# rokulkarni15/distributed-llm-training-inference

Hardware: AMD Instinct MI355X
Metric: train tok/s Llama-2-7B ZeRO-3+LoRA at 1/2/4/8 GPUs; serve tok/s + p50 TTFT (higher is better)
Workload: dtype bf16

## Files before the change

lumen/csrc/kernels/flash_attn.hip:

```cpp
#include "api.h"
#include "common.h"
#include <cstdlib>

namespace lumen {
namespace fa {

typedef __bf16 bf16x8 __attribute__((ext_vector_type(8)));
typedef _Float16 f16x8 __attribute__((ext_vector_type(8)));
typedef float f32x4 __attribute__((ext_vector_type(4)));
typedef short s16x4 __attribute__((ext_vector_type(4)));
typedef __attribute__((address_space(3))) s16x4 lds_s16x4;

constexpr int D = 128;
constexpr int BN = 64;
constexpr int IMG = BN * D * 2;

template <typename T> struct Mfma;
template <> struct Mfma<bf16> {
  static __device__ __forceinline__ f32x4 run(uint4 a, uint4 b, f32x4 c) {
    return __builtin_amdgcn_mfma_f32_16x16x32_bf16(__builtin_bit_cast(bf16x8, a),
                                                   __builtin_bit_cast(bf16x8, b), c, 0, 0, 0);
  }
};
template <> struct Mfma<fp16> {
  static __device__ __forceinline__ f32x4 run(uint4 a, uint4 b, f32x4 c) {
    return __builtin_amdgcn_mfma_f32_16x16x32_f16(__builtin_bit_cast(f16x8, a),
                                                  __builtin_bit_cast(f16x8, b), c, 0, 0, 0);
  }
};

__device__ __forceinline__ int swz(int row) { return ((row & 3) << 2) | ((row >> 2) & 3); }
__device__ __forceinline__ int img_off(int row, int chunk) {
  return row * 256 + ((chunk ^ swz(row)) << 4);
}
template <int SW>
__device__ __forceinline__ int swz_t(int row) {
  if constexpr (SW == 0) return swz(row);
  else return ((row & 1) << 3) | ((row & 2) << 1) | ((row & 4) >> 1);
}
__device__ __forceinline__ unsigned lds_off_g(const char* p) {
  return static_cast<unsigned>(
      reinterpret_cast<uintptr_t>((__attribute__((address_space(3))) const char*)(p)));
}
template <int SW>
__device__ __forceinline__ int img_off_t(int row, int chunk) {
  return row * 256 + ((chunk ^ swz_t<SW>(row)) << 4);
}

template <typename T>
__device__ __forceinline__ void stage64(char* img, const T* base, long long ld, int r0, int rmax) {
#pragma unroll
  for (int i = 0; i < 4; ++i) {
    const int idx = threadIdx.x + i * 256;
    const int row = idx >> 4, ch = idx & 15;
    uint4 v = make_uint4(0, 0, 0, 0);
    if (r0 + row < rmax) v = *reinterpret_cast<const uint4*>(base + (long long)(r0 + row) * ld + ch * 8);
    *reinterpret_cast<uint4*>(img + img_off(row, ch)) = v;
  }
}

template <typename T, int SW = 0>
__device__ __forceinline__ void stage64_async(char* img, const T* base, long long ld, int r0,
                                              int rmax) {
  const int lane = threadIdx.x & 63, wid = threadIdx.x >> 6;
#pragma unroll
  for (int i = 0; i < 4; ++i) {
    const int row = (wid * 4 + i) * 4 + (lane >> 4);
    const int ch = (lane & 15) ^ swz_t<SW>(row);
    int gr = r0 + row;
    gr = gr < rmax ? gr : rmax - 1;
    __builtin_amdgcn_global_load_lds(
        (const void*)(base + (long long)gr * ld + ch * 8),
        (__attribute__((address_space(3))) void*)(img + (wid * 4 + i) * 1024), 16, 0, 0);
  }
}

template <typename T>
__device__ __forceinline__ void stage64_async_s(char* img, const T* base, long long ld, int r0,
                                                int rmax) {
  const int lane = threadIdx.x & 63, wid = __builtin_amdgcn_readfirstlane(threadIdx.x >> 6);
  const char* tile = reinterpret_cast<const char*>(base + (long long)r0 * ld);
  const int last = rmax - 1 - r0;
#pragma unroll
  for (int i = 0; i < 4; ++i) {
    const int row = (wid * 4 + i) * 4 + (lane >> 4);
    const int ch = (lane & 15) ^ swz(row);
    const unsigned off = (unsigned)((row < last ? row : last) * (int)ld + ch * 8) * sizeof(T);
    __builtin_amdgcn_global_load_lds(
        (const void*)(tile + off),
        (__attribute__((address_space(3))) void*)(img + (wid * 4 + i) * 1024), 16, 0, 0);
  }
}

__device__ __forceinline__ void dma16_o(const void* g, const char* lds_wave_base) {
  const unsigned m0 = __builtin_amdgcn_readfirstlane(lds_off_g(lds_wave_base));
  asm volatile("s_mov_b32 m0, %1\n\ts_nop 0\n\tglobal_load_lds_dwordx4 %0, off"
               :: "v"(g), "s"(m0) : "memory", "m0");
}
__device__ __forceinline__ void dma4_o(const void* g, const char* lds_wave_base) {
  const unsigned m0 = __builtin_amdgcn_readfirstlane(lds_off_g(lds_wave_base));
  asm volatile("s_mov_b32 m0, %1\n\ts_nop 0\n\tglobal_load_lds_dword %0, off"
               :: "v"(g), "s"(m0) : "memory", "m0");
}
template <typename T, int SW>
__device__ __forceinline__ void stage64_async_o(char* img, const T* base, long long ld, int r0,
                                                int rmax) {
  const int lane = threadIdx.x & 63, wid = __builtin_amdgcn_readfirstlane(threadIdx.x >> 6);
#pragma unroll
  for (int i = 0; i < 4; ++i) {
    const int row = (wid * 4 + i) * 4 + (lane >> 4);
    const int ch = (lane & 15) ^ swz_t<SW>(row);
    int gr = r0 + row;
    gr = gr < rmax ? gr : rmax - 1;
    dma16_o(base + (long long)gr * ld + ch * 8, img + (wid * 4 + i) * 1024);
  }
}

template <typename T, int SW>
__device__ __forceinline__ void stage64_async8_o(char* img, const T* base, long long ld, int r0,
                                                 int rmax) {
  const int lane = threadIdx.x & 63, wid = threadIdx.x >> 6;
#pragma unroll
  for (int i = 0; i < 2; ++i) {
    const int row = (wid * 2 + i) * 4 + (lane >> 4);
    const int ch = (lane & 15) ^ swz_t<SW>(row);
    int gr = r0 + row;
    gr = gr < rmax ? gr : rmax - 1;
    dma16_o(base + (long long)gr * ld + ch * 8, img + (wid * 2 + i) * 1024);
  }
}

template <typename T>
__device__ __forceinline__ void stage64_paged(char* img, const T* cache, int kvh, int nkv,
                                              const int* bt, int bs, int r0, int rmax) {
  const int lane = threadIdx.x & 63, wid = threadIdx.x >> 6;
#pragma unroll
  for (int i = 0; i < 4; ++i) {
    const int row = (wid * 4 + i) * 4 + (lane >> 4);
    const int ch = (lane & 15) ^ swz(row);
    int gr = r0 + row;
    gr = gr < rmax ? gr : rmax - 1;
    const long long blk = bt[gr / bs];
    const T* src = cache + ((blk * nkv + kvh) * bs + gr % bs) * D + ch * 8;
    __builtin_amdgcn_global_load_lds(
        (const void*)src, (__attribute__((address_space(3))) void*)(img + (wid * 4 + i) * 1024),
        16, 0, 0);
  }
}

__device__ __forceinline__ void wait_vm_all() { __builtin_amdgcn_s_waitcnt(0xF70); }
__device__ __forceinline__ void wait_vm_8() { __builtin_amdgcn_s_waitcnt(0xF78); }
__device__ __forceinline__ void lds_fence_barrier() {
  asm volatile("s_waitcnt lgkmcnt(0)" ::: "memory");
  __builtin_amdgcn_s_barrier();
  asm volatile("" ::: "memory");
}

template <int SW = 0>
__device__ __forceinline__ uint4 row_read(const char* img, int row, int chunk) {
  return *reinterpret_cast<const uint4*>(img + img_off_t<SW>(row, chunk));
}

__device__ __forceinline__ uint2 tr_read_raw(const char* p) {
  s16x4 r = __builtin_amdgcn_ds_read_tr16_b64_v4i16((lds_s16x4*)(p));
  return __builtin_bit_cast(uint2, r);
}

__device__ __forceinline__ uint4 tr_read_img(const char* img, int k0, int n0, int lane) {
  const int L = lane & 15, g = lane >> 4;
  const int col = n0 + 4 * (L & 3);
  const int ch = col >> 3, half = (col >> 2) & 1;
  const int r = k0 + 8 * g + (L >> 2);
  const uint2 lo = tr_read_raw(img + img_off(r, ch) + 8 * half);
  const uint2 hi = tr_read_raw(img + img_off(r + 4, ch) + 8 * half);
  return make_uint4(lo.x, lo.y, hi.x, hi.y);
}

__device__ __forceinline__ uint4 tr_read_y(const char* y, int cols, int k0, int m0, int lane) {
  const int L = lane & 15, g = lane >> 4;
  const int r = k0 + 8 * g + (L >> 2);
  const int c = m0 + 4 * (L & 3);
  const int ld = cols + 4;
  const uint2 lo = tr_read_raw(y + (r * ld + c) * 2);
  const uint2 hi = tr_read_raw(y + ((r + 4) * ld + c) * 2);
  return make_uint4(lo.x, lo.y, hi.x, hi.y);
}

template <typename T>
__device__ __forceinline__ void y_store(char* y, int cols, int k0, int m0, int lane, float v0,
                                        float v1, float v2, float v3) {
  T t[4] = {from_f32<T>(v0), from_f32<T>(v1), from_f32<T>(v2), from_f32<T>(v3)};
  *reinterpret_cast<uint2*>(y + ((k0 + (lane & 15)) * (cols + 4) + m0 + 4 * (lane >> 4)) * 2) =
      *reinterpret_cast<uint2*>(t);
}

template <typename T>
__device__ __forceinline__ uint4 gload16(const T* p, bool ok) {
  return ok ? *reinterpret_cast<const uint4*>(p) : make_uint4(0, 0, 0, 0);
}

template <int CTRL>
__device__ __forceinline__ float dpp(float v) {
  return __builtin_bit_cast(float, __builtin_amdgcn_update_dpp(0, __builtin_bit_cast(int, v), CTRL,
                                                               0xF, 0xF, false));
}
__device__ __forceinline__ float red16_max(float v) {
  v = fmaxf(v, dpp<0xB1>(v));
  v = fmaxf(v, dpp<0x4E>(v));
  v = fmaxf(v, dpp<0x141>(v));
  v = fmaxf(v, dpp<0x140>(v));
  return v;
}
__device__ __forceinline__ float red16_sum(float v) {
  v += dpp<0xB1>(v);
  v += dpp<0x4E>(v);
  v += dpp<0x141>(v);
  v += dpp<0x140>(v);
  return v;
}

__device__ __forceinline__ float fexp2(float x) { return __builtin_amdgcn_exp2f(x); }

struct Args {
  const void* q; const void* k; const void* v;
  long long ldq, ldk, ldv;
  void* o; long long ldo;
  float* lse;
  const int* cu;
  const int* tiles;
  int nh, nkv, T;
  float scale, scale_log2;
  const void* dout; long long lddo;
  void* dq; void* dk; void* dv; long long lddq, lddk, lddv;
  const float* delta;
  const int* rope_pos;
  const float* rope_cos;
  const float* rope_sin;
  const int* kv_lens;
  const int* block_tables;
  int bt_stride;
  int block_size;
  void* ds;
  const int* ds_off;
  int ds_total;
  int tiles3;
  int nitems;
  int snake;
};

struct Work { int seq, r0, head; };
__device__ __forceinline__ Work work_item(const Args& a) {
  if (a.tiles3) {
    const int* t = a.tiles + 3 * blockIdx.x;
    return Work{t[0], t[1], t[2]};
  }
  return Work{a.tiles[2 * blockIdx.x], a.tiles[2 * blockIdx.x + 1], (int)blockIdx.y};
}

__device__ __forceinline__ void rope_inv_pair(float& lo, float& hi, float c, float s) {
  const float l = lo, h = hi;
  lo = l * c + h * s;
  hi = h * c - l * s;
}

template <int SW = 0>
__device__ __forceinline__ uint4 tr_read_img2(const char* img, int rlo, int rhi, int n0, int lane) {
  const int L = lane & 15;
  const int col = n0 + 4 * (L & 3);
  const int ch = col >> 3, half = (col >> 2) & 1;
  const uint2 lo = tr_read_raw(img + img_off_t<SW>(rlo + (L >> 2), ch) + 8 * half);
  const uint2 hi = tr_read_raw(img + img_off_t<SW>(rhi + (L >> 2), ch) + 8 * half);
  return make_uint4(lo.x, lo.y, hi.x, hi.y);
}

template <typename T>
__device__ __forceinline__ uint4 pack_p(const f32x4& a, const f32x4& b) {
  return make_uint4(pk2<T>(a[0], a[1]), pk2<T>(a[2], a[3]), pk2<T>(b[0], b[1]), pk2<T>(b[2], b[3]));
}

template <typename T>
__global__ void __launch_bounds__(256) delta_kernel(Args a) {
  const int lane = threadIdx.x & 63;
  const int t = blockIdx.x * 4 + (threadIdx.x >> 6);
  if (t >= a.T) return;
  const int H = a.nh * D;
  const T* dO = reinterpret_cast<const T*>(a.dout) + (long long)t * a.lddo;
  const T* O = reinterpret_cast<const T*>(a.o) + (long long)t * a.ldo;
  for (int base = 0; base < H; base += 512) {
    const int e = base + lane * 8;
    float s = 0.f;
    if (e < H) {
      float x[8], y[8];
      load8(dO + e, x);
      load8(O + e, y);
#pragma unroll
      for (int j = 0; j < 8; ++j) s += x[j] * y[j];
    }
#pragma unroll
    for (int o = 1; o < 16; o <<= 1) s += __shfl_xor(s, o, 16);
    if ((lane & 15) == 0 && e < H) const_cast<float*>(a.delta)[(long long)(e / D) * a.T + t] = s;
  }
}

__device__ __forceinline__ int ds_slot(int m, int lr) { return (m * 16 + (lr ^ ((m & 1) << 3))) * 16; }
__device__ __forceinline__ long long ds_tile(const Args& a, int head, int seq_base, int qt, int kt,
// ... 305 lines not shown
    vr[1][n] = tr32a<1>(vb, off, n);
    vr[2][n] = tr32a<2>(vb, off, n);
    vr[3][n] = tr32a<3>(vb, off, n);
  }
  float mx = -INFINITY;
#pragma unroll
  for (int kb = 0; kb < 2; ++kb)
#pragma unroll
    for (int r = 0; r < 16; ++r) {
      if (MASK) {
        const int kpos = kv0 + kb * 32 + 8 * (r >> 2) + 4 * hi + (r & 3);
        const bool out = (kpos >= L) | (CAUSAL & (kpos > qrow));
        st[kb][r] = out ? -INFINITY : st[kb][r];
      }
      mx = fmaxf(mx, st[kb][r]);
    }
  mx = xor32_max(mx) * scale_log2;
  constexpr float RESCALE = 8.f;
  const bool bump = mx > m_i + RESCALE;
  if (__any(bump)) {
    const float alpha = bump ? fexp2(m_i - mx) : 1.f;
    const float m_new = bump ? mx : m_i;
    l_i *= alpha;
#pragma unroll
    for (int n = 0; n < 4; ++n) acc[n] *= alpha;
    m_i = m_new;
  }
  const float mref = m_i == -INFINITY ? 0.f : m_i;
  float rs = 0.f;
#pragma unroll
  for (int kb = 0; kb < 2; ++kb)
#pragma unroll
    for (int r = 0; r < 16; ++r) {
      const float p = fexp2(fmaf(st[kb][r], scale_log2, -mref));
      st[kb][r] = p;
      rs += p;
    }
  l_i += xor32_sum(rs);
  const uint4 pb[4] = {pack8<T>(st[0], 0), pack8<T>(st[0], 1), pack8<T>(st[1], 0),
                       pack8<T>(st[1], 1)};
#pragma unroll
  for (int sl = 0; sl < 4; ++sl) {
    lgkm_wait(vr[sl][0], vr[sl][1], vr[sl][2], vr[sl][3]);
#pragma unroll
    for (int n = 0; n < 4; ++n) acc[n] = Mfma32<T>::run(as_u4(vr[sl][n]), pb[sl], acc[n]);
  }
}

template <typename T, bool CAUSAL, bool PAGED = false>
__global__ void __launch_bounds__(256, CAUSAL ? 2 : 1) fwd32_kernel(Args a) {
  constexpr int BM = 128;
  __shared__ __attribute__((aligned(16))) char bufA[2 * IMG];
  __shared__ __attribute__((aligned(16))) char bufB[2 * IMG];
  const int lane = threadIdx.x & 63, wid = threadIdx.x >> 6;
  const int lq = lane & 31, hi = lane >> 5;
  auto run = [&](const int seq, const int q0, const int head) {
  const int kvh = head / (a.nh / a.nkv);
  const int s0 = a.cu[seq], L = a.cu[seq + 1] - s0;
  const int Lk = PAGED ? a.kv_lens[seq] : L;
  const int qoff = Lk - L;
  const T* Q = reinterpret_cast<const T*>(a.q) + (long long)s0 * a.ldq + head * D;
  const T* K = reinterpret_cast<const T*>(a.k) + (PAGED ? 0 : (long long)s0 * a.ldk + kvh * D);
  const T* V = reinterpret_cast<const T*>(a.v) + (PAGED ? 0 : (long long)s0 * a.ldv + kvh * D);
  const int* bt = PAGED ? a.block_tables + (long long)seq * a.bt_stride : nullptr;
  const int wq0 = q0 + wid * 32;
  const int qrow = wq0 + lq;
  const int qpos = qrow + qoff;
  Off32 off;
  make_off32(off, lane);
  f32x16 acc[4];
#pragma unroll
  for (int n = 0; n < 4; ++n) acc[n] = zero16();
  float m_i = -INFINITY, l_i = 0.f;
  const int kv_end = CAUSAL ? min(Lk, q0 + qoff + BM) : Lk;
  const int w_end = CAUSAL ? min(kv_end, wq0 + qoff + 32) : kv_end;
  auto stage = [&](char* img, int r0) {
    if constexpr (PAGED) {
      stage64_paged(img, K, kvh, a.nkv, bt, a.block_size, r0, Lk);
      stage64_paged(img + IMG, V, kvh, a.nkv, bt, a.block_size, r0, Lk);
    } else {
      stage64_async_s(img, K, a.ldk, r0, L);
      stage64_async_s(img + IMG, V, a.ldv, r0, L);
    }
  };
  uint4 qf[8];
  {
    const bool two = q0 + 64 < L;
    stage64_async_s(bufB, Q, a.ldq, q0, L);
    if (two) stage64_async_s(bufB + IMG, Q, a.ldq, q0 + 64, L);
    if (kv_end > 0) {
      stage(bufA, 0);
      wait_vm_8();
    } else {
      wait_vm_all();
    }
    __builtin_amdgcn_s_barrier();
    asm volatile("" ::: "memory");
    const int r = 32 * wid + lq;
    const char* qi = bufB + (r >> 6) * IMG;
#pragma unroll
    for (int ks = 0; ks < 8; ++ks) qf[ks] = row_read(qi, r & 63, 2 * ks + hi);
    lds_fence_barrier();
  }
  auto tile = [&](char* cur, char* nxt, int kv0) {
    if (kv0 + BN < kv_end) {
      stage(nxt, kv0 + BN);
      wait_vm_8();
    } else {
      wait_vm_all();
    }
    lds_fence_barrier();
    if (kv0 < w_end) {
      const bool need_mask = (kv0 + BN > Lk) || (CAUSAL && kv0 + BN - 1 > wq0 + qoff);
      if (need_mask)
        fwd32_tile<T, CAUSAL, true>(cur, cur + IMG, off, qf, acc, m_i, l_i, kv0, Lk, qpos,
                                           hi, a.scale_log2);
      else
        fwd32_tile<T, CAUSAL, false>(cur, cur + IMG, off, qf, acc, m_i, l_i, kv0, Lk, qpos,
                                            hi, a.scale_log2);
    }
    lds_fence_barrier();
  };
  for (int kv0 = 0; kv0 < kv_end; kv0 += 2 * BN) {
    tile(bufA, bufB, kv0);
    if (kv0 + BN < kv_end) tile(bufB, bufA, kv0 + BN);
  }
  {
    int ln = threadIdx.x;
    asm volatile("" : "+v"(ln));
    const int lq2 = ln & 31, hi2 = (ln >> 5) & 1;
    const float inv = l_i > 0.f ? 1.f / l_i : 0.f;
    char* ot = bufA + wid * 8192;
#pragma unroll
    for (int n = 0; n < 4; ++n)
#pragma unroll
      for (int j = 0; j < 4; ++j) {
        struct alignas(8) O4 { T v[4]; } o4;
#pragma unroll
        for (int i = 0; i < 4; ++i) o4.v[i] = from_f32<T>(acc[n][4 * j + i] * inv);
        *reinterpret_cast<O4*>(ot + img_off(lq2, 4 * n + j) + 8 * hi2) = o4;
      }
    if (hi == 0 && a.lse && qrow < L)
      a.lse[(long long)head * a.T + s0 + qrow] = l_i > 0.f ? m_i + __log2f(l_i) : INFINITY;
    asm volatile("s_waitcnt lgkmcnt(0)" ::: "memory");
    T* O = reinterpret_cast<T*>(a.o) + (long long)s0 * a.ldo + head * D;
    const int ch = ln & 15;
#pragma unroll
    for (int it = 0; it < 8; ++it) {
      const int r = 4 * it + ((ln >> 4) & 3);
      const uint4 v = *reinterpret_cast<const uint4*>(ot + img_off(r, ch));
      if (wq0 + r < L) *reinterpret_cast<uint4*>(O + (long long)(wq0 + r) * a.ldo + ch * 8) = v;
    }
  }
  if (a.nitems > 0) lds_fence_barrier();
  };
  if (a.nitems > 0) {
    const int G = gridDim.x, w = blockIdx.x;
    for (int base = 0; base < a.nitems; base += G) {
      const int it = (a.snake && ((base / G) & 1)) ? base + G - 1 - w : base + w;
      if (it >= a.nitems) continue;
      const int ti = it / a.nh;
      run(a.tiles[2 * ti], a.tiles[2 * ti + 1], it - ti * a.nh);
    }
  } else {
    const Work wk = work_item(a);
    if (wk.seq < 0) return;
    run(wk.seq, wk.r0, wk.head);
  }
}


template <typename T, bool CAUSAL, bool MASK>
__device__ __forceinline__ void dq32_tile(const char* kimg, const char* vimg, const Off32& off,
                                          const uint4 (&qf)[8], const uint4 (&of)[8],
                                          f32x16 (&dq)[4], int kv0, int L, int qrow, int hi,
                                          float lse_q, float del_q, float scale_log2) {
#pragma unroll
  for (int kb = 0; kb < 2; ++kb) {
    f32x16 st = zero16(), dpt = zero16();
#pragma unroll
    for (int ks = 0; ks < 8; ++ks) {
      st = Mfma32<T>::run(lds16(kimg + kb * 8192 + off.row[ks]), qf[ks], st);
      dpt = Mfma32<T>::run(lds16(vimg + kb * 8192 + off.row[ks]), of[ks], dpt);
    }
#pragma unroll
    for (int r = 0; r < 16; ++r) {
      float pv = fexp2(fmaf(st[r], scale_log2, -lse_q));
      if (MASK) {
        const int kpos = kv0 + kb * 32 + 8 * (r >> 2) + 4 * hi + (r & 3);
        const bool out = (kpos >= L) | (qrow >= L) | (CAUSAL & (kpos > qrow));
        pv = out ? 0.f : pv;
      }
      dpt[r] = pv * (dpt[r] - del_q);
    }
#pragma unroll
    for (int s = 0; s < 2; ++s) {
      const uint4 db = pack8<T>(dpt, s);
#pragma unroll
      for (int n = 0; n < 4; ++n)
        dq[n] = Mfma32<T>::run(tr32(kimg, off, kb * 32 + 16 * s, n), db, dq[n]);
    }
  }
}

template <typename T, bool CAUSAL>
__global__ void __launch_bounds__(256, 2) bwd_dq32_kernel(Args a) {
  constexpr int BM = 128;
  __shared__ __attribute__((aligned(16))) char smem[4 * IMG];
  const int lane = threadIdx.x & 63, wid = threadIdx.x >> 6;
  const int lq = lane & 31, hi = lane >> 5;
  const Work wk = work_item(a);
  if (wk.seq < 0) return;
  const int seq = wk.seq, q0 = wk.r0;
  const int head = wk.head, kvh = head / (a.nh / a.nkv);
  const int s0 = a.cu[seq], L = a.cu[seq + 1] - s0;
  const T* Q = reinterpret_cast<const T*>(a.q) + (long long)s0 * a.ldq + head * D;
  const T* dO = reinterpret_cast<const T*>(a.dout) + (long long)s0 * a.lddo + head * D;
  const T* K = reinterpret_cast<const T*>(a.k) + (long long)s0 * a.ldk + kvh * D;
  const T* V = reinterpret_cast<const T*>(a.v) + (long long)s0 * a.ldv + kvh * D;
  const int wq0 = q0 + wid * 32;
  const int qrow = wq0 + lq;
  uint4 qf[8], of[8];
#pragma unroll
  for (int ks = 0; ks < 8; ++ks) {
    qf[ks] = gload16(Q + (long long)qrow * a.ldq + 16 * ks + 8 * hi, qrow < L);
    of[ks] = gload16(dO + (long long)qrow * a.lddo + 16 * ks + 8 * hi, qrow < L);
  }
  const float lse_q = qrow < L ? a.lse[(long long)head * a.T + s0 + qrow] : INFINITY;
  const float del_q = qrow < L ? a.delta[(long long)head * a.T + s0 + qrow] : 0.f;
  f32x16 dq[4];
#pragma unroll
  for (int n = 0; n < 4; ++n) dq[n] = zero16();
  const int kv_end = CAUSAL ? min(L, q0 + BM) : L;
  const int w_end = CAUSAL ? min(kv_end, wq0 + 32) : kv_end;
  wait_vm_all();
  if (kv_end > 0) {
    stage64_async(smem, K, a.ldk, 0, L);
    stage64_async(smem + IMG, V, a.ldv, 0, L);
  }
  Off32 off;
  make_off32(off, lane);
  int it = 0;
  for (int kv0 = 0; kv0 < kv_end; kv0 += BN, ++it) {
    char* kimg = smem + (it & 1) * 2 * IMG;
    char* vimg = kimg + IMG;
    if (kv0 + BN < kv_end) {
      char* nk = smem + ((it + 1) & 1) * 2 * IMG;
      stage64_async(nk, K, a.ldk, kv0 + BN, L);
      stage64_async(nk + IMG, V, a.ldv, kv0 + BN, L);
      wait_vm_8();
    } else {
      wait_vm_all();
    }
    lds_fence_barrier();
    if (kv0 < w_end) {
      const bool need_mask = (kv0 + BN > L) || (wq0 + 32 > L) || (CAUSAL && kv0 + BN - 1 > wq0);
      if (need_mask)
        dq32_tile<T, CAUSAL, true>(kimg, vimg, off, qf, of, dq, kv0, L, qrow, hi, lse_q, del_q,
                                   a.scale_log2);
      else
        dq32_tile<T, CAUSAL, false>(kimg, vimg, off, qf, of, dq, kv0, L, qrow, hi, lse_q, del_q,
                                    a.scale_log2);
    }
    lds_fence_barrier();
  }
  if (qrow < L) {
    T* dQ = reinterpret_cast<T*>(a.dq) + (long long)s0 * a.lddq + head * D + (long long)qrow * a.lddq;
#pragma unroll
    for (int n = 0; n < 4; ++n)
#pragma unroll
      for (int r = 0; r < 16; ++r) dq[n][r] *= a.scale;
    if (a.rope_pos != nullptr) {
      const float* cb = a.rope_cos + (long long)a.rope_pos[s0 + qrow] * 64 + 4 * hi;
      const float* sb = a.rope_sin + (long long)a.rope_pos[s0 + qrow] * 64 + 4 * hi;
#pragma unroll
      for (int n = 0; n < 2; ++n)
#pragma unroll
        for (int jj = 0; jj < 4; ++jj) {
          const float4 c4 = *reinterpret_cast<const float4*>(cb + 32 * n + 8 * jj);
          const float4 s4 = *reinterpret_cast<const float4*>(sb + 32 * n + 8 * jj);
          const float cs[4] = {c4.x, c4.y, c4.z, c4.w}, sn[4] = {s4.x, s4.y, s4.z, s4.w};
#pragma unroll
          for (int i = 0; i < 4; ++i) {
            float lo = dq[n][4 * jj + i], hi2 = dq[n + 2][4 * jj + i];
            rope_inv_pair(lo, hi2, cs[i], sn[i]);
            dq[n][4 * jj + i] = lo;
            dq[n + 2][4 * jj + i] = hi2;
          }
        }
    }
#pragma unroll
    for (int n = 0; n < 4; ++n)
#pragma unroll
      for (int jj = 0; jj < 4; ++jj) {
        struct alignas(8) O4 { T v[4]; } q4;
#pragma unroll
        for (int i = 0; i < 4; ++i) q4.v[i] = from_f32<T>(dq[n][4 * jj + i]);
        *reinterpret_cast<O4*>(dQ + 32 * n + 8 * jj + 4 * hi) = q4;
      }
  }
}

template <typename T, bool CAUSAL>
__global__ void __launch_bounds__(256) bwd_dq_ds_kernel(Args a) {
  constexpr int TILE = IMG + 8192;
  __shared__ __attribute__((aligned(16))) char bufA[TILE];
  __shared__ __attribute__((aligned(16))) char bufB[TILE];
  const int lane = threadIdx.x & 63, wid = __builtin_amdgcn_readfirstlane(threadIdx.x >> 6);
  const int lr = lane & 15, lg = lane >> 4;
  auto run = [&](const int seq, const int q0, const int head) {
  const int kvh = head / (a.nh / a.nkv);
  const int s0 = a.cu[seq], L = a.cu[seq + 1] - s0;
  const int ns = (L + 63) / 64, qt = q0 / 64;
  const T* K = reinterpret_cast<const T*>(a.k) + (long long)s0 * a.ldk + kvh * D;
  const char* dsq = reinterpret_cast<const char*>(a.ds) + ds_tile(a, head, a.ds_off[seq], qt, 0, ns, CAUSAL);
  const int nkt = CAUSAL ? qt + 1 : ns;
  const int si = lr >> 2, sm = lr & 3;
  const int dso = ((wid >> 1) * 1024) + (wid & 1) * 8 + ds_slot(sm, 4 * lg + si);
  auto stage = [&](char* buf, int kt) {
    stage64_async_o<T, 1>(buf, K, a.ldk, kt * 64, L);
    const char* src = dsq + (long long)kt * 8192;
#pragma unroll
    for (int i = 0; i < 2; ++i) {
      const int off = (wid * 2 + i) * 1024;
      dma16_o(src + off + lane * 16, buf + IMG + off);
    }
  };
  f32x4 dq[8];
#pragma unroll
  for (int n = 0; n < 8; ++n) dq[n] = f32x4{0.f, 0.f, 0.f, 0.f};
  if (nkt > 0) stage(bufA, 0);
  auto step = [&](int kt, char* buf, char* nx) {
    if (kt + 1 < nkt) {
      stage(nx, kt + 1);
      asm volatile("s_waitcnt vmcnt(6)" ::: "memory");
    } else {
      wait_vm_all();
    }
    lds_fence_barrier();
    const char* kimg = buf;
    const char* dsi = buf + IMG;
#pragma unroll
    for (int ks = 0; ks < 2; ++ks) {
      const uint2 lo = tr_read_raw(dsi + (2 * ks) * 2048 + dso);
      const uint2 hi = tr_read_raw(dsi + (2 * ks + 1) * 2048 + dso);
      const uint4 af = make_uint4(lo.x, lo.y, hi.x, hi.y);
#pragma unroll
      for (int n = 0; n < 8; ++n)
        dq[n] = Mfma<T>::run(af, tr_read_img2<1>(kimg, 32 * ks + 4 * lg, 32 * ks + 16 + 4 * lg, n * 16, lane), dq[n]);
    }
    lds_fence_barrier();
  };
  for (int kt = 0; kt < nkt; kt += 2) {
    step(kt, bufA, bufB);
    if (kt + 1 < nkt) step(kt + 1, bufB, bufA);
  }
  T* dQ = reinterpret_cast<T*>(a.dq) + (long long)s0 * a.lddq + head * D;
#pragma unroll
  for (int r = 0; r < 4; ++r) {
    const int qr = q0 + wid * 16 + 4 * lg + r;
    if (qr >= L) continue;
    float qv[8];
#pragma unroll
    for (int n = 0; n < 8; ++n) qv[n] = dq[n][r] * a.scale;
    if (a.rope_pos != nullptr) {
      const long long pb = (long long)a.rope_pos[s0 + qr] * 64 + lr;
#pragma unroll
      for (int n = 0; n < 4; ++n)
        rope_inv_pair(qv[n], qv[n + 4], a.rope_cos[pb + 16 * n], a.rope_sin[pb + 16 * n]);
    }
#pragma unroll
    for (int n = 0; n < 8; ++n) dQ[(long long)qr * a.lddq + n * 16 + lr] = from_f32<T>(qv[n]);
  }
  };
  if (a.nitems > 0) {
    const int G = gridDim.x, w = blockIdx.x;
    for (int base = 0; base < a.nitems; base += G) {
      const int it = (a.snake && ((base / G) & 1)) ? base + G - 1 - w : base + w;
      if (it >= a.nitems) continue;
      const int ti = it / a.nh;
      run(a.tiles[2 * ti], a.tiles[2 * ti + 1], it - ti * a.nh);
    }
  } else {
    const Work wk = work_item(a);
    if (wk.seq < 0) return;
    run(wk.seq, wk.r0, wk.head);
  }
}


static int cu_count() {
  static int n = [] {
    int dev = 0, v = 0;
    if (hipGetDevice(&dev) != hipSuccess ||
        hipDeviceGetAttribute(&v, hipDeviceAttributeMultiprocessorCount, dev) != hipSuccess || v <= 0)
      v = 256;
    return v;
  }();
  return n;
}

template <typename T>
static hipError_t launch(int which, int causal, int mt, int ntiles, const Args& a, hipStream_t st) {
  dim3 block(256);
  if (which == 0) {
    if (mt != 20) return hipErrorInvalidValue;
    dim3 grid(ntiles, a.tiles3 ? 1 : a.nh);
    if (a.nitems > 0) grid = dim3(std::min(a.nitems, (causal ? 2 : 1) * cu_count()), 1);
    if (causal) hipLaunchKernelGGL((fwd32_kernel<T, true>), grid, block, 0, st, a);
    else hipLaunchKernelGGL((fwd32_kernel<T, false>), grid, block, 0, st, a);
  } else if (which == 1) {
    dim3 grid((unsigned)((a.T + 3) / 4));
    hipLaunchKernelGGL(delta_kernel<T>, grid, block, 0, st, a);
  } else if (which == 2) {
    dim3 grid(ntiles, a.tiles3 ? 1 : a.nkv);
    if (causal) hipLaunchKernelGGL((bwd_dkdv_kernel<T, true>), grid, block, 0, st, a);
    else hipLaunchKernelGGL((bwd_dkdv_kernel<T, false>), grid, block, 0, st, a);
  } else if (which == 5) {
    dim3 grid(ntiles, a.tiles3 ? 1 : a.nh);
    if (causal) hipLaunchKernelGGL((bwd_dq32_kernel<T, true>), grid, block, 0, st, a);
    else hipLaunchKernelGGL((bwd_dq32_kernel<T, false>), grid, block, 0, st, a);
  } else if (which == 7) {
    dim3 grid(ntiles, a.tiles3 ? 1 : a.nkv);
    if (a.nitems > 0) grid = dim3(std::min(a.nitems, 2 * cu_count()), 1);
    if (causal) hipLaunchKernelGGL((bwd_dkdv_kernel<T, true, true>), grid, block, 0, st, a);
    else hipLaunchKernelGGL((bwd_dkdv_kernel<T, false, true>), grid, block, 0, st, a);
  } else if (which == 8) {
    dim3 grid(ntiles, a.tiles3 ? 1 : a.nh);
    if (a.nitems > 0) grid = dim3(std::min(a.nitems, 3 * cu_count()), 1);
    if (causal) hipLaunchKernelGGL((bwd_dq_ds_kernel<T, true>), grid, block, 0, st, a);
    else hipLaunchKernelGGL((bwd_dq_ds_kernel<T, false>), grid, block, 0, st, a);
  } else if (which == 6) {
    dim3 grid(ntiles, a.nh);
    if (a.nitems > 0) grid = dim3(std::min(a.nitems, (causal ? 2 : 1) * cu_count()), 1);
    if (causal) hipLaunchKernelGGL((fwd32_kernel<T, true, true>), grid, block, 0, st, a);
    else hipLaunchKernelGGL((fwd32_kernel<T, false, true>), grid, block, 0, st, a);
  } else {
    return hipErrorInvalidValue;
  }
  return hipGetLastError();
}

}
}

#include <algorithm>
#include <cstdlib>
static int fa_persist() {
  static int v = [] { const char* e = std::getenv("LUMEN_FA_PERSIST"); return e ? std::atoi(e) : 15; }();
  return v;
}

extern "C" hipError_t lumen_flash_attn(int dtype, int which, int causal, int mt,
                                       const void* q, const void* k, const void* v,
                                       long long ldq, long long ldk, long long ldv, void* o,
                                       long long ldo, float* lse, const int* cu,
                                       const int* tiles, int ntiles, int nh, int nkv, int T,
                                       float scale, const void* dout, long long lddo, void* dq,
                                       void* dk, void* dv, long long lddq, long long lddk,
                                       long long lddv, const float* delta, const int* rope_pos,
                                       const float* rope_cos, const float* rope_sin,
                                       hipStream_t st) {
  if (nkv <= 0 || nh % nkv != 0) return hipErrorInvalidValue;
  const int tiles3 = (which >> 8) & 1;
  which &= 0xff;
  if (tiles3 && which != 0 && which != 2 && which != 5) return hipErrorInvalidValue;
  if (rope_pos != nullptr && which != 2 && which != 5) return hipErrorInvalidValue;
  if (which != 1 && ntiles == 0) return hipSuccess;
  lumen::fa::Args a;
  a.q = q; a.k = k; a.v = v; a.ldq = ldq; a.ldk = ldk; a.ldv = ldv; a.o = o; a.ldo = ldo;
  a.lse = lse; a.cu = cu; a.tiles = tiles; a.nh = nh; a.nkv = nkv; a.T = T;
  a.scale = scale; a.scale_log2 = scale * 1.4426950408889634f;
  a.dout = dout; a.lddo = lddo; a.dq = dq; a.dk = dk; a.dv = dv; a.lddq = lddq; a.lddk = lddk;
  a.lddv = lddv; a.delta = delta;
  a.rope_pos = rope_pos; a.rope_cos = rope_cos; a.rope_sin = rope_sin;
  a.kv_lens = nullptr; a.block_tables = nullptr; a.bt_stride = 0; a.block_size = 0;
  a.ds = nullptr; a.ds_off = nullptr; a.ds_total = 0; a.tiles3 = tiles3;
  a.nitems = (which == 0 && mt == 20 && !tiles3 && (fa_persist() & 2)) ? ntiles * nh : 0;
  a.snake = (fa_persist() >> 3) & 1;
  if (which == 6 || which == 7 || which == 8) return hipErrorInvalidValue;
  if (dtype == lumen::kBF16) return lumen::fa::launch<lumen::bf16>(which, causal, mt, ntiles, a, st);
  if (dtype == lumen::kF16) return lumen::fa::launch<lumen::fp16>(which, causal, mt, ntiles, a, st);
  return hipErrorInvalidValue;
}

extern "C" hipError_t lumen_flash_attn_paged(int dtype, int causal, const void* q, long long ldq,
                                             const void* k_cache, const void* v_cache, void* o,
                                             long long ldo, const int* cu_q, const int* kv_lens,
                                             const int* tiles, int ntiles,
                                             const int* block_tables, int bt_stride,
                                             int block_size, int nh, int nkv, int T, float scale,
                                             hipStream_t st) {
  if (nkv <= 0 || nh % nkv != 0 || block_size <= 0) return hipErrorInvalidValue;
  if (ntiles == 0) return hipSuccess;
  lumen::fa::Args a{};
  a.q = q; a.ldq = ldq; a.k = k_cache; a.v = v_cache; a.ldk = a.ldv = 0;
  a.o = o; a.ldo = ldo; a.lse = nullptr; a.cu = cu_q; a.tiles = tiles;
  a.nh = nh; a.nkv = nkv; a.T = T;
  a.scale = scale; a.scale_log2 = scale * 1.4426950408889634f;
  a.kv_lens = kv_lens; a.block_tables = block_tables; a.bt_stride = bt_stride;
  a.block_size = block_size;
  a.nitems = 0;
  if (dtype == lumen::kBF16) return lumen::fa::launch<lumen::bf16>(6, causal, 20, ntiles, a, st);
  if (dtype == lumen::kF16) return lumen::fa::launch<lumen::fp16>(6, causal, 20, ntiles, a, st);
  return hipErrorInvalidValue;
}

extern "C" hipError_t lumen_flash_attn_ds(int dtype, int which, int causal, const void* q,
                                          const void* k, const void* v, long long ldq,
                                          long long ldk, long long ldv, const float* lse,
                                          const int* cu, const int* tiles, int ntiles, int nh,
                                          int nkv, int T, float scale, const void* dout,
                                          long long lddo, void* dq, void* dk, void* dv,
                                          long long lddq, long long lddk, long long lddv,
                                          const float* delta, const int* rope_pos,
                                          const float* rope_cos, const float* rope_sin, void* ds,
                                          const int* ds_off, int ds_total, hipStream_t st) {
  const int tiles3 = (which >> 8) & 1;
  which &= 0xff;
  if (nkv <= 0 || nh % nkv != 0 || (which != 7 && which != 8) || ds == nullptr ||
      ds_off == nullptr)
    return hipErrorInvalidValue;
  if (ntiles == 0) return hipSuccess;
  lumen::fa::Args a{};
  a.q = q; a.k = k; a.v = v; a.ldq = ldq; a.ldk = ldk; a.ldv = ldv;
  a.lse = const_cast<float*>(lse); a.cu = cu; a.tiles = tiles; a.nh = nh; a.nkv = nkv; a.T = T;
  a.scale = scale; a.scale_log2 = scale * 1.4426950408889634f;
  a.dout = dout; a.lddo = lddo; a.dq = dq; a.dk = dk; a.dv = dv; a.lddq = lddq; a.lddk = lddk;
  a.lddv = lddv; a.delta = delta;
  a.rope_pos = rope_pos; a.rope_cos = rope_cos; a.rope_sin = rope_sin;
  a.ds = ds; a.ds_off = ds_off; a.ds_total = ds_total; a.tiles3 = tiles3;
  a.snake = (fa_persist() >> 3) & 1;
  a.nitems = tiles3 ? 0 : (which == 7 && (fa_persist() & 1)) ? ntiles * nkv
                        : (which == 8 && (fa_persist() & 4)) ? ntiles * nh : 0;
  if (dtype == lumen::kBF16) return lumen::fa::launch<lumen::bf16>(which, causal, 1, ntiles, a, st);
  if (dtype == lumen::kF16) return lumen::fa::launch<lumen::fp16>(which, causal, 1, ntiles, a, st);
  return hipErrorInvalidValue;
}
```

lumen/ops/attention.py:

```python
from __future__ import annotations

import math
import os
from typing import Optional

import torch
import torch.nn.functional as F

from ._native import native, use_native
from .quant import MX_BLOCK, Mxfp4Weight, quantize_mxfp4_rows


def causal_attention(q: torch.Tensor, k: torch.Tensor, v: torch.Tensor,
                     scale: Optional[float] = None) -> torch.Tensor:
    B, nh, S, D = q.shape
    nkv = k.shape[1]
    if nkv != nh:
        if q.is_cuda:
            o = F.scaled_dot_product_attention(q, k, v, is_causal=True, scale=scale,
                                               enable_gqa=True)
        else:
            rep = nh // nkv
            o = F.scaled_dot_product_attention(q, k.repeat_interleave(rep, 1),
                                               v.repeat_interleave(rep, 1), is_causal=True,
# ... 95 lines not shown
            to = torch.empty(num_seqs, nh, max_parts, D, device=q.device, dtype=torch.float32)
        else:
            tm = torch.empty(1, 1, 1, device=q.device, dtype=torch.float32)
            tl, to = tm, tm
        one = PA_ONE_PASS if one_pass is None else int(one_pass)
        fused = bool(fused_merge) and not one
        cnt = (_pa_counters(q.device, num_seqs * nkv) if fused and max_parts > 1
               else None)
        qk = q if (q.stride(2) == 1 and q.stride(1) == D and q.stride(0) % D == 0
                   and q.data_ptr() % 16 == 0) else q.contiguous()
        native().paged_attention_decode(out, qk, _kv_buf(k_cache), _kv_buf(v_cache), block_tables,
                                        context_lens, nkv, bs, block_tables.shape[1], scale, tm,
                                        tl, to, partition_size, cnt, one)
        return out
    return paged_decode_ref(q, k_cache, v_cache, block_tables, context_lens, scale)


def paged_decode_ref(q, k_cache, v_cache, block_tables, context_lens, scale):
    num_seqs, nh, D = q.shape
    nkv, bs = k_cache.shape[1], k_cache.shape[2]
    g = nh // nkv
    out = torch.empty_like(q)
    for i in range(num_seqs):
        L = int(context_lens[i])
        nblk = (L + bs - 1) // bs
        blks = block_tables[i, :nblk].long()
        kk = _kv_gather_f32(k_cache, blks).permute(1, 0, 2, 3).reshape(nkv, nblk * bs, D)[:, :L]
        vv = _kv_gather_f32(v_cache, blks).permute(1, 0, 2, 3).reshape(nkv, nblk * bs, D)[:, :L]
        qq = q[i].float().view(nkv, g, D)
        s = torch.einsum("hgd,hld->hgl", qq, kk) * scale
        p = torch.softmax(s, -1)
        out[i] = torch.einsum("hgl,hld->hgd", p, vv).reshape(nh, D).to(q.dtype)
    return out


def flash_attention_paged(q: torch.Tensor, k_cache: torch.Tensor, v_cache: torch.Tensor,
                          cu_q, kv_lens, block_tables: torch.Tensor, nh: int, nkv: int,
                          D: int, scale: Optional[float] = None,
                          out: Optional[torch.Tensor] = None) -> torch.Tensor:
    T = q.shape[0]
    scale = scale if scale is not None else 1.0 / math.sqrt(D)
    if out is None:
        out = torch.empty(T, nh * D, device=q.device, dtype=q.dtype)
    if use_native(q) and D == 128 and k_cache.shape[-1] == 128:
        cu = tuple(int(c) for c in cu_q)
        dev = q.device
        cut = _cu_tensor(cu, dev)
        kl = (kv_lens if isinstance(kv_lens, torch.Tensor)
              else torch.tensor(list(kv_lens), dtype=torch.int32, device=dev))
        kl = kl.to(torch.int32)
        bt = block_tables.to(torch.int32)
        if isinstance(k_cache, Mxfp4KV) or k_cache.dtype == FP8_KV:
            k_cache, v_cache, bt = _dequant_blocks(k_cache, v_cache, bt, kl, q.dtype)
        native().flash_attn_paged(True, q, k_cache, v_cache, out, cut, kl,
                                  _tiles(cu, 128, dev), bt, nh, nkv, scale)
        return out
    out.copy_(flash_attention_paged_ref(q, k_cache, v_cache, cu_q, kv_lens, block_tables, nh,
                                        nkv, D, scale))
    return out


FP8_KV = torch.float8_e4m3fn
_SCRATCH: dict = {}


def _dequant_blocks(k_cache, v_cache, bt, kv_lens, dtype):
    P, maxb = bt.shape
    nb, nkv, bs, D = k_cache.shape
    need = P * maxb
    key = (k_cache.device, dtype, nkv, bs, D)
    scr = _SCRATCH.get(key)
    if scr is None or scr[0].shape[0] < need:
        n = max(need, 256)
        scr = (torch.empty(n, nkv, bs, D, device=k_cache.device, dtype=dtype),
               torch.empty(n, nkv, bs, D, device=k_cache.device, dtype=dtype),
               torch.arange(n, device=k_cache.device, dtype=torch.int32))
        _SCRATCH[key] = scr
    ks, vs, ident = scr
    if isinstance(k_cache, Mxfp4KV):
        native().kv_dequant_mx(k_cache.buf, v_cache.buf, ks, vs, bt, kv_lens, maxb)
    else:
        native().kv_dequant(k_cache, v_cache, ks, vs, bt, kv_lens, maxb)
    return ks, vs, ident[:need].view(P, maxb)


def flash_attention_paged_ref(q, k_cache, v_cache, cu_q, kv_lens, block_tables, nh, nkv, D,
                              scale=None):
    scale = scale if scale is not None else 1.0 / math.sqrt(D)
    cu = [int(c) for c in cu_q]
    kl = [int(x) for x in kv_lens]
    bs = k_cache.shape[2]
    g = nh // nkv
    outs = []
    for s in range(len(kl)):
        a, b = cu[s], cu[s + 1]
        n, L = b - a, kl[s]
        nblk = (L + bs - 1) // bs
        blks = block_tables[s, :nblk].long()
        kk = _kv_gather_f32(k_cache, blks).permute(1, 0, 2, 3).reshape(nkv, nblk * bs, D)[:, :L]
        vv = _kv_gather_f32(v_cache, blks).permute(1, 0, 2, 3).reshape(nkv, nblk * bs, D)[:, :L]
        qq = q[a:b, :nh * D].float().view(n, nkv, g, D)
        sc = torch.einsum("nhgd,hld->hgnl", qq, kk) * scale
        qpos = torch.arange(L - n, L, device=q.device)[:, None]
        kpos = torch.arange(L, device=q.device)[None, :]
        sc = sc.masked_fill(kpos > qpos, float("-inf"))
        p = torch.softmax(sc, -1)
        o = torch.einsum("hgnl,hld->nhgd", p, vv).reshape(n, nh * D)
        outs.append(o.to(q.dtype))
    return torch.cat(outs, 0) if outs else q.new_zeros(0, nh * D)


def write_kv_cache(k: torch.Tensor, v: torch.Tensor, k_cache: torch.Tensor,
                   v_cache: torch.Tensor, slot_mapping: torch.Tensor) -> None:
    T = slot_mapping.numel()
    if T == 0:
        return
    nb, nkv, bs, D = k_cache.shape
    if use_native(_kv_buf(k_cache)):
        native().reshape_and_cache(k, v, _kv_buf(k_cache), _kv_buf(v_cache), slot_mapping, nkv,
                                   D, bs, k.stride(0), v.stride(0))
        return
    sm = slot_mapping.long()
    valid = sm >= 0
    sm = sm[valid]
    blk, off = sm // bs, sm % bs
    if isinstance(k_cache, Mxfp4KV):
        k_cache.write(k[valid], blk, off)
        v_cache.write(v[valid], blk, off)
        return
    k_cache[blk, :, off] = k[valid].to(k_cache.dtype)
    v_cache[blk, :, off] = v[valid].to(v_cache.dtype)


def rope_write_kv(qkv: torch.Tensor, positions: torch.Tensor, nh: int, nkv: int, D: int,
                  cos_t: torch.Tensor, sin_t: torch.Tensor, k_cache: torch.Tensor,
                  v_cache: torch.Tensor, slot_mapping: torch.Tensor) -> None:
    T = qkv.shape[0]
    if T == 0:
        return
    nb, nkv_c, bs, Dc = k_cache.shape
    if (use_native(qkv) and D % 16 == 0 and nkv_c == nkv and Dc == D
            and (not isinstance(k_cache, Mxfp4KV) or D == 32 or D % 64 == 0)):
        native().rope_cache_write(qkv, positions.to(torch.int32), cos_t, sin_t, _kv_buf(k_cache),
                                  _kv_buf(v_cache), slot_mapping.to(torch.int64), nh, nkv, D, bs)
        return
    from .rope import rope_inplace

    rope_inplace(qkv, positions, nh + nkv, D, cos_t, sin_t)
    qs, ks = nh * D, nkv * D
    write_kv_cache(qkv[:, qs:qs + ks].view(T, nkv, D), qkv[:, qs + ks:qs + 2 * ks].view(T, nkv, D),
                   k_cache, v_cache, slot_mapping)



_TILE_CACHE = {}


def _upload_i32(vals, device) -> torch.Tensor:
    h = torch.tensor(vals, dtype=torch.int32)
    if torch.device(device).type != "cuda":
        return h
    return h.pin_memory().to(device, non_blocking=True)


def _tiles(cu: tuple, rows: int, device, heavy_first: bool = True,
           heavy_low: bool = False) -> torch.Tensor:
    key = (cu, rows, str(device), heavy_first, heavy_low)
    t = _TILE_CACHE.get(key)
    if t is None:
        lst = []
        for s in range(len(cu) - 1):
            L = cu[s + 1] - cu[s]
            lst += [(s, r) for r in range(0, L, rows)]
        if heavy_low:
            lst.sort(key=lambda x: (x[1], -(cu[x[0] + 1] - cu[x[0]])))
        elif heavy_first:
            lst.sort(key=lambda x: -x[1])
        t = _upload_i32(lst if lst else [(0, 0)], device).reshape(-1)
        if not lst:
            t = t[:0]
        if len(_TILE_CACHE) > 256:
            _TILE_CACHE.clear()
        _TILE_CACHE[key] = t
    return t


def _cu_tensor(cu: tuple, device) -> torch.Tensor:
    key = ("cu", cu, str(device))
    t = _TILE_CACHE.get(key)
    if t is None:
        t = _upload_i32(list(cu), device)
        _TILE_CACHE[key] = t
    return t


def prepare_varlen(cu: tuple, device) -> None:
    rows_set = (FA_FWD_ROWS, 64, 128)
    keys = ([("cu", cu, str(device))] + [(cu, r, str(device), True, False) for r in rows_set]
            + [(cu, 64, str(device), True, True)])
    if all(k in _TILE_CACHE for k in keys):
        return
    parts = [list(cu)]
    for rows, low in [(r, False) for r in rows_set] + [(64, True)]:
        lst = []
        for s in range(len(cu) - 1):
            lst += [(s, r) for r in range(0, cu[s + 1] - cu[s], rows)]
        if low:
            lst.sort(key=lambda x: (x[1], -(cu[x[0] + 1] - cu[x[0]])))
        else:
            lst.sort(key=lambda x: -x[1])
        parts.append([v for t in lst for v in t])
    flat = torch.tensor([v for p in parts for v in p], dtype=torch.int32)
    if torch.cuda.is_available():
        flat = flat.pin_memory()
    dev = flat.to(device, non_blocking=True)
    if len(_TILE_CACHE) > 256:
        _TILE_CACHE.clear()
    o = 0
    for k, p in zip(keys, parts):
        _TILE_CACHE[k] = dev[o:o + len(p)]
        o += len(p)
    _TILE_CACHE[("pin", cu, str(device))] = flat


import os as _os
FA_FWD_MT, FA_FWD_ROWS = 20, 128
FA_DS_MB = float(_os.environ.get("LUMEN_FA_DS_MB", "2048"))


def _ds_offsets(cu: tuple, causal: bool, device):
    key = ("ds", cu, causal, str(device))
    hit = _TILE_CACHE.get(key)
    if hit is None:
        offs, tot = [], 0
        for s in range(len(cu) - 1):
            n = (cu[s + 1] - cu[s] + 63) // 64
            offs.append(tot)
            tot += n * (n + 1) // 2 if causal else n * n
        hit = (torch.tensor(offs if offs else [0], dtype=torch.int32, device=device), tot)
        _TILE_CACHE[key] = hit
    return hit


DELTA_HANDOFFS = [0]


class _FlashAttn(torch.autograd.Function):
    @staticmethod
    def forward(ctx, qkv, cu, nh, nkv, D, causal, rope=None, scale=None, out_ext=0):
        C = native()
        T = qkv.shape[0]
        q = qkv[:, :nh * D]
        k = qkv[:, nh * D:(nh + nkv) * D]
        v = qkv[:, (nh + nkv) * D:]
        o = torch.empty(T, nh * D + out_ext, device=qkv.device, dtype=qkv.dtype)[:, :nh * D]
        lse = torch.empty(nh, T, device=qkv.device, dtype=torch.float32)
        cut = _cu_tensor(cu, qkv.device)
        scale = 1.0 / math.sqrt(D) if scale is None else scale
        tl = _tiles(cu, FA_FWD_ROWS, qkv.device)
        C.flash_attn(0, causal, FA_FWD_MT, q, k, v, o, lse, cut, tl, nh, nkv, scale, None, None,
                     None, None, None, None, None, None)
        ctx.save_for_backward(qkv, o, lse)
        ctx.meta = (cu, nh, nkv, D, causal, scale)
        ctx.rope = rope
        ctx.delta_slot = {}
        o._lumen_delta_slot = ctx.delta_slot
        return o

    @staticmethod
    def backward(ctx, do):
        C = native()
        qkv, o, lse = ctx.saved_tensors
        cu, nh, nkv, D, causal, scale = ctx.meta
        do = do.contiguous()
        T = qkv.shape[0]
        q = qkv[:, :nh * D]
        k = qkv[:, nh * D:(nh + nkv) * D]
        v = qkv[:, (nh + nkv) * D:]
        dqkv = torch.empty_like(qkv)
        dqkv._lumen_scratch = True
        dq = dqkv[:, :nh * D]
        dk = dqkv[:, nh * D:(nh + nkv) * D]
        dv = dqkv[:, (nh + nkv) * D:]
        slot = ctx.delta_slot
        handed = (slot.get("key") == (do.data_ptr(), do._version)
                  and tuple(slot["delta"].shape) == (nh, T))
        delta = (slot.pop("delta") if handed
                 else torch.empty(nh, T, device=qkv.device, dtype=torch.float32))
        DELTA_HANDOFFS[0] += int(handed)
        slot.clear()
        cut = _cu_tensor(cu, qkv.device)
        wkv, rkv, wq, rq = 2, 64, 5, 128
        rp = ctx.rope
        pos, cos, sin = rp if rp is not None else (None, None, None)
        qtiles = _tiles(cu, rq, qkv.device)
        ds_off, ds_total = (_ds_offsets(cu, causal, qkv.device) if FA_DS_MB > 0
                            else (None, 0))
        if ds_off is not None and nh * ds_total * 8192 <= FA_DS_MB * 2 ** 20:
            ds = torch.empty(nh, ds_total, 4096, device=qkv.device, dtype=qkv.dtype)
            if not handed:
                C.flash_attn(1, causal, 1, q, k, v, o, lse, cut, _tiles(cu, 64, qkv.device), nh,
                             nkv, scale, do, None, None, None, delta, None, None, None)
            t7 = _tiles(cu, 64, qkv.device, heavy_low=causal)
            t8 = _tiles(cu, 64, qkv.device)
            C.flash_attn_ds(7, causal, q, k, v, lse, cut, t7, nh, nkv,
                            scale, do, dq, dk, dv, delta, ds, ds_off, ds_total, pos, cos, sin)
            C.flash_attn_ds(8, causal, q, k, v, lse, cut, t8, nh, nkv,
                            scale, do, dq, dk, dv, delta, ds, ds_off, ds_total, pos, cos, sin)
        else:
            if not handed:
                C.flash_attn(1, causal, 1, q, k, v, o, lse, cut, _tiles(cu, 64, qkv.device), nh,
                             nkv, scale, do, None, None, None, delta, None, None, None)
            C.flash_attn(wkv, causal, 1, q, k, v, o, lse, cut, _tiles(cu, rkv, qkv.device), nh,
                         nkv, scale, do, dq, dk, dv, delta, pos, cos, sin)
            C.flash_attn(wq, causal, 1, q, k, v, o, lse, cut, qtiles, nh, nkv,
                         scale, do, dq, dk, dv, delta, pos, cos, sin)
        if rp is not None:
            dqkv._lumen_rope_undone = True
        return dqkv, None, None, None, None, None, None, None, None


KERNEL_D = 128


def _flash_padded(qkv, cu, nh, nkv, D, causal):
    T = qkv.shape[0]
    H3 = nh + 2 * nkv
    qkvp = F.pad(qkv.view(T, H3, D), (0, KERNEL_D - D)).view(T, H3 * KERNEL_D)
    o = _FlashAttn.apply(qkvp, cu, nh, nkv, KERNEL_D, causal, None, 1.0 / math.sqrt(D))
    return o.view(T, nh, KERNEL_D)[:, :, :D].reshape(T, nh * D)


def flash_attention_qkv(qkv: torch.Tensor, cu_seqlens, nh: int, nkv: int, D: int,
                        causal: bool = True, rope=None, out_ext: int = 0) -> torch.Tensor:
    cu = tuple(int(c) for c in cu_seqlens)
    if use_native(qkv) and D == KERNEL_D:
        return _FlashAttn.apply(qkv, cu, nh, nkv, D, causal, rope, None, out_ext)
    if use_native(qkv) and D < KERNEL_D and D % 8 == 0 and rope is None:
        return _flash_padded(qkv.contiguous(), cu, nh, nkv, D, causal)
    return flash_attention_ref(qkv, cu, nh, nkv, D, causal)


def flash_attention_fresh(qkv: torch.Tensor, cu, nh: int, nkv: int, D: int, scale: float,
                          out: torch.Tensor) -> torch.Tensor:
    cu = tuple(int(c) for c in cu)
    T = qkv.shape[0]
    q = qkv[:, :nh * D]
    k = qkv[:, nh * D:(nh + nkv) * D]
    v = qkv[:, (nh + nkv) * D:(nh + 2 * nkv) * D]
    lse = torch.empty(nh, T, device=qkv.device, dtype=torch.float32)
    native().flash_attn(0, True, FA_FWD_MT, q, k, v, out, lse, _cu_tensor(cu, qkv.device),
                        _tiles(cu, FA_FWD_ROWS, qkv.device), nh, nkv, scale, None, None, None,
                        None, None, None, None, None)
    return out


def flash_attention_ref(qkv, cu, nh, nkv, D, causal=True):
    outs = []
    for s in range(len(cu) - 1):
        a, b = cu[s], cu[s + 1]
        n = b - a
        q = qkv[a:b, :nh * D].view(n, nh, D).transpose(0, 1)[None]
        k = qkv[a:b, nh * D:(nh + nkv) * D].view(n, nkv, D).transpose(0, 1)[None]
        v = qkv[a:b, (nh + nkv) * D:].view(n, nkv, D).transpose(0, 1)[None]
        if nkv != nh:
            rep = nh // nkv
            k, v = k.repeat_interleave(rep, 1), v.repeat_interleave(rep, 1)
        o = F.scaled_dot_product_attention(q, k, v, is_causal=causal)
        outs.append(o[0].transpose(0, 1).reshape(n, nh * D))
    return torch.cat(outs, 0)
```

Before: 45060.

## Process two query tiles per dQ-from-dS block to reuse staged K tiles

The dQ-from-stored-dS backward kernel now handles 128 query rows (two 64-row tiles) per work item, staging two dS tiles alongside each K tile and reusing every K fragment read from LDS for two MFMA accumulations. The aim is to halve K global loads and LDS transposed reads per dQ row and reduce the number of work items. In exchange it doubles the accumulator registers and dS LDS buffers, declares launch bounds for 2 blocks per CU, and lowers the persistent grid from 3x to 2x the CU count. Under causal masking, the last K tile only feeds the second query tile. The Python side passes the 128-row q-tile list to this kernel.

```diff
diff --git a/lumen/csrc/kernels/flash_attn.hip b/lumen/csrc/kernels/flash_attn.hip
--- a/lumen/csrc/kernels/flash_attn.hip
+++ b/lumen/csrc/kernels/flash_attn.hip
@@ -1,6 +1,7 @@
 #include "api.h"
 #include "common.h"
 #include <cstdlib>
+#include <type_traits>
 
 namespace lumen {
 namespace fa {
@@ -912,8 +913,8 @@
 }
 
 template <typename T, bool CAUSAL>
-__global__ void __launch_bounds__(256) bwd_dq_ds_kernel(Args a) {
-  constexpr int TILE = IMG + 8192;
+__global__ void __launch_bounds__(256, 2) bwd_dq_ds_kernel(Args a) {
+  constexpr int TILE = IMG + 2 * 8192;
   __shared__ __attribute__((aligned(16))) char bufA[TILE];
   __shared__ __attribute__((aligned(16))) char bufB[TILE];
   const int lane = threadIdx.x & 63, wid = __builtin_amdgcn_readfirstlane(threadIdx.x >> 6);
@@ -921,44 +922,75 @@
   auto run = [&](const int seq, const int q0, const int head) {
   const int kvh = head / (a.nh / a.nkv);
   const int s0 = a.cu[seq], L = a.cu[seq + 1] - s0;
-  const int ns = (L + 63) / 64, qt = q0 / 64;
+  const int ns = (L + 63) / 64, qt0 = q0 / 64;
+  const bool has1 = qt0 + 1 < ns;
   const T* K = reinterpret_cast<const T*>(a.k) + (long long)s0 * a.ldk + kvh * D;
-  const char* dsq = reinterpret_cast<const char*>(a.ds) + ds_tile(a, head, a.ds_off[seq], qt, 0, ns, CAUSAL);
-  const int nkt = CAUSAL ? qt + 1 : ns;
+  const int ds_base = a.ds_off[seq];
+  const char* ds0 = reinterpret_cast<const char*>(a.ds) + ds_tile(a, head, ds_base, qt0, 0, ns, CAUSAL);
+  const char* ds1 = has1 ? reinterpret_cast<const char*>(a.ds) + ds_tile(a, head, ds_base, qt0 + 1, 0, ns, CAUSAL)
+                         : ds0;
+  const int nkt = CAUSAL ? qt0 + 1 + (has1 ? 1 : 0) : ns;
   const int si = lr >> 2, sm = lr & 3;
   const int dso = ((wid >> 1) * 1024) + (wid & 1) * 8 + ds_slot(sm, 4 * lg + si);
   auto stage = [&](char* buf, int kt) {
     stage64_async_o<T, 1>(buf, K, a.ldk, kt * 64, L);
-    const char* src = dsq + (long long)kt * 8192;
+    const char* src0 = ((CAUSAL && kt > qt0) ? ds1 : ds0) + (long long)kt * 8192;
+    const char* src1 = ds1 + (long long)kt * 8192;
 #pragma unroll
     for (int i = 0; i < 2; ++i) {
       const int off = (wid * 2 + i) * 1024;
-      dma16_o(src + off + lane * 16, buf + IMG + off);
+      dma16_o(src0 + off + lane * 16, buf + IMG + off);
+      dma16_o(src1 + off + lane * 16, buf + IMG + 8192 + off);
     }
   };
-  f32x4 dq[8];
-#pragma unroll
-  for (int n = 0; n < 8; ++n) dq[n] = f32x4{0.f, 0.f, 0.f, 0.f};
+  f32x4 dq[2][8];
+#pragma unroll
+  for (int h = 0; h < 2; ++h)
+#pragma unroll
+    for (int n = 0; n < 8; ++n) dq[h][n] = f32x4{0.f, 0.f, 0.f, 0.f};
+  int rp[2][4];
+  if (a.rope_pos != nullptr) {
+#pragma unroll
+    for (int h = 0; h < 2; ++h)
+#pragma unroll
+      for (int r = 0; r < 4; ++r) {
+        const int qr = q0 + 64 * h + wid * 16 + 4 * lg + r;
+        rp[h][r] = a.rope_pos[s0 + (qr < L ? qr : L - 1)];
+      }
+  }
   if (nkt > 0) stage(bufA, 0);
+  auto products = [&](const char* buf, auto H0, auto H1) {
+    const char* kimg = buf;
+    const char* dsi = buf + IMG;
+#pragma unroll
+    for (int ks = 0; ks < 2; ++ks) {
+      uint4 af[2];
+#pragma unroll
+      for (int h = 0; h < 2; ++h) {
+        if ((h == 0 && !decltype(H0)::value) || (h == 1 && !decltype(H1)::value)) continue;
+        const uint2 lo = tr_read_raw(dsi + h * 8192 + (2 * ks) * 2048 + dso);
+        const uint2 hi = tr_read_raw(dsi + h * 8192 + (2 * ks + 1) * 2048 + dso);
+        af[h] = make_uint4(lo.x, lo.y, hi.x, hi.y);
+      }
+#pragma unroll
+      for (int n = 0; n < 8; ++n) {
+        const uint4 kf = tr_read_img2<1>(kimg, 32 * ks + 4 * lg, 32 * ks + 16 + 4 * lg, n * 16, lane);
+        if constexpr (decltype(H0)::value) dq[0][n] = Mfma<T>::run(af[0], kf, dq[0][n]);
+        if constexpr (decltype(H1)::value) dq[1][n] = Mfma<T>::run(af[1], kf, dq[1][n]);
+      }
+    }
+  };
   auto step = [&](int kt, char* buf, char* nx) {
     if (kt + 1 < nkt) {
       stage(nx, kt + 1);
-      asm volatile("s_waitcnt vmcnt(6)" ::: "memory");
+      asm volatile("s_waitcnt vmcnt(8)" ::: "memory");
     } else {
       wait_vm_all();
     }
     lds_fence_barrier();
-    const char* kimg = buf;
-    const char* dsi = buf + IMG;
-#pragma unroll
-    for (int ks = 0; ks < 2; ++ks) {
-      const uint2 lo = tr_read_raw(dsi + (2 * ks) * 2048 + dso);
-      const uint2 hi = tr_read_raw(dsi + (2 * ks + 1) * 2048 + dso);
-      const uint4 af = make_uint4(lo.x, lo.y, hi.x, hi.y);
-#pragma unroll
-      for (int n = 0; n < 8; ++n)
-        dq[n] = Mfma<T>::run(af, tr_read_img2<1>(kimg, 32 * ks + 4 * lg, 32 * ks + 16 + 4 * lg, n * 16, lane), dq[n]);
-    }
+    if (!has1) products(buf, std::true_type{}, std::false_type{});
+    else if (CAUSAL && kt > qt0) products(buf, std::false_type{}, std::true_type{});
+    else products(buf, std::true_type{}, std::true_type{});
     lds_fence_barrier();
   };
   for (int kt = 0; kt < nkt; kt += 2) {
@@ -967,21 +999,23 @@
   }
   T* dQ = reinterpret_cast<T*>(a.dq) + (long long)s0 * a.lddq + head * D;
 #pragma unroll
-  for (int r = 0; r < 4; ++r) {
-    const int qr = q0 + wid * 16 + 4 * lg + r;
-    if (qr >= L) continue;
-    float qv[8];
-#pragma unroll
-    for (int n = 0; n < 8; ++n) qv[n] = dq[n][r] * a.scale;
-    if (a.rope_pos != nullptr) {
-      const long long pb = (long long)a.rope_pos[s0 + qr] * 64 + lr;
-#pragma unroll
-      for (int n = 0; n < 4; ++n)
-        rope_inv_pair(qv[n], qv[n + 4], a.rope_cos[pb + 16 * n], a.rope_sin[pb + 16 * n]);
-    }
-#pragma unroll
-    for (int n = 0; n < 8; ++n) dQ[(long long)qr * a.lddq + n * 16 + lr] = from_f32<T>(qv[n]);
-  }
+  for (int h = 0; h < 2; ++h)
+#pragma unroll
+    for (int r = 0; r < 4; ++r) {
+      const int qr = q0 + 64 * h + wid * 16 + 4 * lg + r;
+      if (qr >= L) continue;
+      float qv[8];
+#pragma unroll
+      for (int n = 0; n < 8; ++n) qv[n] = dq[h][n][r] * a.scale;
+      if (a.rope_pos != nullptr) {
+        const long long pb = (long long)rp[h][r] * 64 + lr;
+#pragma unroll
+        for (int n = 0; n < 4; ++n)
+          rope_inv_pair(qv[n], qv[n + 4], a.rope_cos[pb + 16 * n], a.rope_sin[pb + 16 * n]);
+      }
+#pragma unroll
+      for (int n = 0; n < 8; ++n) dQ[(long long)qr * a.lddq + n * 16 + lr] = from_f32<T>(qv[n]);
+    }
   };
   if (a.nitems > 0) {
     const int G = gridDim.x, w = blockIdx.x;
@@ -1037,7 +1071,7 @@
     else hipLaunchKernelGGL((bwd_dkdv_kernel<T, false, true>), grid, block, 0, st, a);
   } else if (which == 8) {
     dim3 grid(ntiles, a.tiles3 ? 1 : a.nh);
-    if (a.nitems > 0) grid = dim3(std::min(a.nitems, 3 * cu_count()), 1);
+    if (a.nitems > 0) grid = dim3(std::min(a.nitems, 2 * cu_count()), 1);
     if (causal) hipLaunchKernelGGL((bwd_dq_ds_kernel<T, true>), grid, block, 0, st, a);
     else hipLaunchKernelGGL((bwd_dq_ds_kernel<T, false>), grid, block, 0, st, a);
   } else if (which == 6) {
diff --git a/lumen/ops/attention.py b/lumen/ops/attention.py
--- a/lumen/ops/attention.py
+++ b/lumen/ops/attention.py
@@ -421,7 +421,7 @@
                 C.flash_attn(1, causal, 1, q, k, v, o, lse, cut, _tiles(cu, 64, qkv.device), nh,
                              nkv, scale, do, None, None, None, delta, None, None, None)
             t7 = _tiles(cu, 64, qkv.device, heavy_low=causal)
-            t8 = _tiles(cu, 64, qkv.device)
+            t8 = qtiles
             C.flash_attn_ds(7, causal, q, k, v, lse, cut, t7, nh, nkv,
                             scale, do, dq, dk, dv, delta, ds, ds_off, ds_total, pos, cos, sin)
             C.flash_attn_ds(8, causal, q, k, v, lse, cut, t8, nh, nkv,
```

New measurement: 45120 (median of 6 runs). No clear change (+0.1%).
